# PaddlePaddle/PaddleScience

Hardware: NVIDIA H100
Metric: collocation-points/sec PDE residual loss+grad (LDC N-S) (higher is better)
Workload: dtype f32

## Files before the change

### paddlescience_b200/csrc/kernels_wgmma.cuh

```cuda
#pragma once

#include "kernels_thin.cuh"

#ifndef PPSCI_EMUL
#include <stdint.h>

namespace ppsci {
namespace wg {

constexpr int KCH = 32;
constexpr int THREADS = 256;
constexpr int TM = 64;
constexpr int A_TILE_BYTES = TM * KCH * 4;
__host__ __device__ inline int tile_points(int C) { return TM / C; }

__host__ __device__ inline int stage_bytes(int N) { return 2 * A_TILE_BYTES + 2 * N * KCH * 4; }
__host__ __device__ inline int fwd_smem_bytes(int N) { return 2 * stage_bytes(N) + 1024 + 64; }
constexpr int PREFETCH_MAX_CS = 8;

__host__ __device__ __forceinline__ uint32_t sw128(int row, int kk) {
  return (uint32_t)(row * 128 + ((((kk >> 2) ^ row) & 7) << 4) + ((kk & 3) << 2));
}
__device__ __forceinline__ uint32_t sw128_q(int row, int kq) { return (uint32_t)(row * 128 + (((kq ^ row) & 7) << 4)); }

__device__ __forceinline__ uint32_t smem_u32(const void* p) { return (uint32_t)__cvta_generic_to_shared(p); }

__device__ __forceinline__ float tf32_rn(float x) {
  uint32_t u;
  asm("cvt.rna.tf32.f32 %0, %1;" : "=r"(u) : "f"(x));
  return __uint_as_float(u);
}

__device__ __forceinline__ void mbar_init(uint32_t bar, uint32_t count) {
  asm volatile("mbarrier.init.shared::cta.b64 [%0], %1;" ::"r"(bar), "r"(count) : "memory");
}
__device__ __forceinline__ void mbar_expect_tx(uint32_t bar, uint32_t bytes) {
  asm volatile("mbarrier.arrive.expect_tx.shared::cta.b64 _, [%0], %1;" ::"r"(bar), "r"(bytes) : "memory");
}
__device__ __forceinline__ bool mbar_try_wait(uint32_t bar, uint32_t parity) {
  uint32_t ok;
  asm volatile(
      "{\n\t.reg .pred p;\n\t"
      "mbarrier.try_wait.parity.shared::cta.b64 p, [%1], %2;\n\t"
      "selp.u32 %0, 1, 0, p;\n\t}"
      : "=r"(ok)
      : "r"(bar), "r"(parity)
      : "memory");
  return ok != 0;
}
__device__ __forceinline__ void mbar_wait(uint32_t bar, uint32_t parity) {
  uint32_t spins = 0;
  while (!mbar_try_wait(bar, parity)) {
    if (++spins > (1u << 26)) __trap();
  }
}
__device__ __forceinline__ void bulk_g2s(uint32_t dst_smem, const void* src, uint32_t bytes, uint32_t bar) {
  asm volatile("cp.async.bulk.shared::cluster.global.mbarrier::complete_tx::bytes [%0], [%1], %2, [%3];" ::"r"(dst_smem),
               "l"(src), "r"(bytes), "r"(bar)
               : "memory");
}
__device__ __forceinline__ void fence_proxy_async() { asm volatile("fence.proxy.async.shared::cta;" ::: "memory"); }

__device__ __forceinline__ uint64_t make_desc(uint32_t saddr) {
  uint64_t d = 0;
  d |= (uint64_t)((saddr & 0x3FFFFu) >> 4);
  d |= (uint64_t)1 << 16;
  d |= (uint64_t)(1024 >> 4) << 32;
  d |= (uint64_t)1 << 62;
  return d;
}
__device__ __forceinline__ void wgmma_fence() { asm volatile("wgmma.fence.sync.aligned;" ::: "memory"); }
__device__ __forceinline__ void wgmma_commit() { asm volatile("wgmma.commit_group.sync.aligned;" ::: "memory"); }
template <int N>
__device__ __forceinline__ void wgmma_wait() {
  asm volatile("wgmma.wait_group.sync.aligned %0;" ::"n"(N) : "memory");
}
#define WG_T0 "%0, %1, %2, %3, %4, %5, %6, %7"
#define WG_T1 WG_T0 ", %8, %9, %10, %11, %12, %13, %14, %15"
#define WG_T2 WG_T1 ", %16, %17, %18, %19, %20, %21, %22, %23"
#define WG_T3 WG_T2 ", %24, %25, %26, %27, %28, %29, %30, %31"
#define WG_T4 WG_T3 ", %32, %33, %34, %35, %36, %37, %38, %39"
#define WG_T5 WG_T4 ", %40, %41, %42, %43, %44, %45, %46, %47"
#define WG_T6 WG_T5 ", %48, %49, %50, %51, %52, %53, %54, %55"
#define WG_T7 WG_T6 ", %56, %57, %58, %59, %60, %61, %62, %63"
#define WG_O8(b) "+f"(d[b]), "+f"(d[b + 1]), "+f"(d[b + 2]), "+f"(d[b + 3]), "+f"(d[b + 4]), "+f"(d[b + 5]), "+f"(d[b + 6]), "+f"(d[b + 7])
#define WG_O0 WG_O8(0)
#define WG_O1 WG_O0, WG_O8(8)
#define WG_O2 WG_O1, WG_O8(16)
#define WG_O3 WG_O2, WG_O8(24)
#define WG_O4 WG_O3, WG_O8(32)
#define WG_O5 WG_O4, WG_O8(40)
#define WG_O6 WG_O5, WG_O8(48)
#define WG_O7 WG_O6, WG_O8(56)
#define WG_MMA(M, G, IA, IB, IP)                                                                                  \
  __device__ __forceinline__ void wgmma_tf32(float (&d)[M / 2], uint64_t da, uint64_t db, uint32_t accumulate) { \
    asm volatile(                                                                                                 \
        "{\n\t.reg .pred p;\n\t"                                                                                  \
        "setp.ne.b32 p, %" #IP ", 0;\n\t"                                                                          \
        "wgmma.mma_async.sync.aligned.m64n" #M "k8.f32.tf32.tf32 {" WG_T##G "}, %" #IA ", %" #IB ", p, 1, 1;\n\t}"  \
        : WG_O##G                                                                                                 \
        : "l"(da), "l"(db), "r"(accumulate));                                                                     \
  }
WG_MMA(16, 0, 8, 9, 10)
WG_MMA(32, 1, 16, 17, 18)
WG_MMA(48, 2, 24, 25, 26)
WG_MMA(64, 3, 32, 33, 34)
WG_MMA(80, 4, 40, 41, 42)
WG_MMA(96, 5, 48, 49, 50)
WG_MMA(112, 6, 56, 57, 58)
WG_MMA(128, 7, 64, 65, 66)
#undef WG_MMA

__global__ void k_wg_prep_w(const float* __restrict__ W, float* __restrict__ img, int K, int N, int transposed) {
  const long long i = (long long)blockIdx.x * blockDim.x + threadIdx.x;
  if (i >= (long long)K * N) return;
  const int n = (int)(i / K), k = (int)(i % K);
  const float w = transposed ? W[(long long)n * K + k] : W[(long long)k * N + n];
  const float hi = tf32_rn(w);
  float* blk = img + (long long)(k / KCH) * 2 * N * KCH;
  const uint32_t off = sw128(n, k % KCH) >> 2;
  blk[off] = hi;
  blk[(long long)N * KCH + off] = w - hi;
}

struct WgArgs {
  AOperand<float> A;
  JetLayout J;
  const float* Wimg;
  int Kdim;
  int Kvalid;
  int Nout;
  const float* bias;
  float* Out;
  int ldo;
  long long oplane;
  long long Np;
  int num_tiles;
  const float* Zprev;
  int ldz;
  long long zplane;
  int act;
};

__device__ __forceinline__ unsigned char* xchg(unsigned char* base_ptr, int sbytes, int N, int r, int col) {
  return base_ptr + sbytes + 2 * A_TILE_BYTES + r * N * 4 + ((((col >> 2) ^ r) & 7) << 4) + (((col >> 2) & ~7) << 4) +
         (col & 3) * 4;
}

template <class L, int NQ, bool DX>
__global__ void __launch_bounds__(THREADS, 1) k_wg_layer(WgArgs g) {
  PPSCI_DYN_SMEM(smem_dyn);
  const uint32_t base = (smem_u32(smem_dyn) + 1023u) & ~1023u;
  unsigned char* base_ptr = smem_dyn + (base - smem_u32(smem_dyn));
  constexpr int CS = L::CS;
  constexpr int TP = TM / CS;
  constexpr int rows_used = CS * TP;
  constexpr int PPR = (THREADS / 32) * 4;
  constexpr int MAXI = (TP + PPR - 1) / PPR;
  constexpr int N = NQ * 32;
  constexpr int NH = N / 2;
  constexpr bool PREFETCH = CS <= PREFETCH_MAX_CS;
  const int sbytes = stage_bytes(N);
  const uint32_t bar0 = base + 2 * sbytes;
  const uint32_t b_bytes = (uint32_t)(2 * N * KCH * 4);
  const int tid = threadIdx.x, warp = tid >> 5, lane = tid & 31, wgi = tid >> 7;
  const int kq = lane & 7, psub = lane >> 3;
  const int nchunks = g.Kdim / KCH;
  const int act = g.A.act;

  if (tid == 0) {
    mbar_init(bar0, 1);
    mbar_init(bar0 + 8, 1);
    asm volatile("fence.mbarrier_init.release.cluster;" ::: "memory");
  }
  for (int s = 0; s < 2; ++s) {
    float4* az = reinterpret_cast<float4*>(base_ptr + s * sbytes);
    for (int i = tid; i < 2 * A_TILE_BYTES / 16; i += THREADS) az[i] = make_float4(0.f, 0.f, 0.f, 0.f);
  }
  fence_proxy_async();
  __syncthreads();

  float4 z[MAXI][CS];
  bool zok[MAXI];
  auto load_z = [&](int tile, int j) {
#pragma unroll
    for (int i = 0; i < MAXI; ++i) {
      const int pl = warp * 4 + psub + i * PPR;
      const long long p = (long long)tile * TP + pl;
      zok[i] = pl < TP && tile < g.num_tiles && p < g.Np;
      if (g.Kvalid && j * KCH + 4 * kq >= g.Kvalid) zok[i] = false;
      const float* src = g.A.Z + p * g.A.ld + j * KCH + 4 * kq;
#pragma unroll
      for (int c = 0; c < CS; ++c)
        z[i][c] = zok[i] ? __ldg(reinterpret_cast<const float4*>(src + (long long)c * g.A.plane)) : make_float4(0.f, 0.f, 0.f, 0.f);
    }
  };
  if constexpr (PREFETCH) load_z(blockIdx.x, 0);

  float ex[NH / 2], cr[NH / 2];
  const int rbase = (warp & 3) * 16 + (lane >> 2);
  const int cbase = wgi * NH + 2 * (lane & 3);
  uint32_t it = 0;
  for (int tile = blockIdx.x; tile < g.num_tiles; tile += gridDim.x) {
    const long long p0 = (long long)tile * TP;
#pragma unroll
    for (int e = 0; e < NH / 2; ++e) ex[e] = cr[e] = 0.f;
    for (int j = 0; j < nchunks; ++j, ++it) {
      const uint32_t s = it & 1u;
      wgmma_wait<1>();
      __syncthreads();
      const uint32_t st_addr = base + s * sbytes;
      unsigned char* st_ptr = base_ptr + s * sbytes;
      if (tid == 0) {
        mbar_expect_tx(bar0 + 8 * s, b_bytes);
        bulk_g2s(st_addr + 2 * A_TILE_BYTES, g.Wimg + (long long)j * 2 * N * KCH, b_bytes, bar0 + 8 * s);
      }
      if constexpr (!PREFETCH) load_z(tile, j);
#pragma unroll
      for (int i = 0; i < MAXI; ++i) {
        const int pl = warp * 4 + psub + i * PPR;
        if (pl >= TP) continue;
        const bool valid = zok[i];
        float yout[CS][4];
        if constexpr (DX) {
#pragma unroll
          for (int c = 0; c < CS; ++c) {
            yout[c][0] = z[i][c].x; yout[c][1] = z[i][c].y; yout[c][2] = z[i][c].z; yout[c][3] = z[i][c].w;
          }
        } else {
#pragma unroll
          for (int t = 0; t < 4; ++t) {
            auto comp = [&](const float4& v) { return t == 0 ? v.x : t == 1 ? v.y : t == 2 ? v.z : v.w; };
            float sc[6];
            float y0;
            act_coef<float, L::KM>(act, comp(z[i][0]), y0, sc);
            yout[0][t] = valid ? y0 : 0.f;
            jet_fwd<float, L>(g.J, sc, [&](int c) { return comp(z[i][c]); }, [&](int c, float v) { yout[c][t] = valid ? v : 0.f; });
          }
        }
#pragma unroll
        for (int c = 0; c < CS; ++c) {
          float4 h, l;
          h.x = tf32_rn(yout[c][0]); h.y = tf32_rn(yout[c][1]); h.z = tf32_rn(yout[c][2]); h.w = tf32_rn(yout[c][3]);
          l.x = yout[c][0] - h.x; l.y = yout[c][1] - h.y; l.z = yout[c][2] - h.z; l.w = yout[c][3] - h.w;
          const uint32_t off = sw128_q(c * TP + pl, kq);
          *reinterpret_cast<float4*>(st_ptr + off) = h;
          *reinterpret_cast<float4*>(st_ptr + A_TILE_BYTES + off) = l;
        }
      }
      if constexpr (PREFETCH) {
        if (j + 1 < nchunks) load_z(tile, j + 1);
        else load_z(tile + gridDim.x, 0);
      }
      fence_proxy_async();
      __syncthreads();
      mbar_wait(bar0 + 8 * s, (it >> 1) & 1u);
      const uint64_t a_hi = make_desc(st_addr), a_lo = make_desc(st_addr + A_TILE_BYTES);
      const uint64_t b_hi = make_desc(st_addr + 2 * A_TILE_BYTES + wgi * NH * 128), b_lo = b_hi + (uint64_t)(N * 128 / 16);
      wgmma_fence();
#pragma unroll
      for (int ks = 0; ks < KCH / 8; ++ks) {
        const uint64_t inc = (uint64_t)(2 * ks);
        const uint32_t first = (j == 0 && ks == 0) ? 0u : 1u;
        wgmma_tf32(ex, a_hi + inc, b_hi + inc, first);
        wgmma_tf32(cr, a_lo + inc, b_hi + inc, first);
        wgmma_tf32(cr, a_hi + inc, b_lo + inc, 1u);
      }
      wgmma_commit();
    }
    wgmma_wait<0>();
    if constexpr (!DX) {
#pragma unroll
      for (int h = 0; h < 2; ++h) {
        const int r = rbase + 8 * h;
        const int c = r / TP, pl = r - c * TP;
        const long long p = p0 + pl;
        if (r >= rows_used || p >= g.Np) continue;
        float* out_row = g.Out + (long long)c * g.oplane + p * g.ldo;
#pragma unroll
        for (int j = 0; j < NH / 8; ++j) {
          const int col = cbase + 8 * j;
          float2 v = make_float2(ex[4 * j + 2 * h] + cr[4 * j + 2 * h], ex[4 * j + 2 * h + 1] + cr[4 * j + 2 * h + 1]);
          if (c == 0 && g.bias) {
            v.x += __ldg(g.bias + col);
            v.y += __ldg(g.bias + col + 1);
          }
          *reinterpret_cast<float2*>(out_row + col) = v;
        }
      }
    } else {
      __syncthreads();
#pragma unroll
      for (int h = 0; h < 2; ++h) {
        const int r = rbase + 8 * h;
#pragma unroll
        for (int j = 0; j < NH / 8; ++j)
          *reinterpret_cast<float2*>(xchg(base_ptr, sbytes, N, r, cbase + 8 * j)) =
              make_float2(ex[4 * j + 2 * h] + cr[4 * j + 2 * h], ex[4 * j + 2 * h + 1] + cr[4 * j + 2 * h + 1]);
      }
      constexpr int N4 = N / 4;
      auto load_zc = [&](int item, float4 (&zc)[CS]) {
        const int pl = item / N4, q = item - pl * N4;
        const long long p = p0 + pl;
        if (item >= TP * N4 || p >= g.Np) return;
#pragma unroll
        for (int c = 0; c < CS; ++c)
          zc[c] = __ldg(reinterpret_cast<const float4*>(g.Zprev + (long long)c * g.zplane + p * g.ldz + 4 * q));
      };
      float4 znext[CS];
      if constexpr (PREFETCH) load_zc(tid, znext);
      __syncthreads();
      for (int item = tid; item < TP * N4; item += THREADS) {
        const int pl = item / N4, q = item - pl * N4;
        const long long p = p0 + pl;
        float4 zc[CS];
        if constexpr (PREFETCH) {
#pragma unroll
          for (int c = 0; c < CS; ++c) zc[c] = znext[c];
          load_zc(item + THREADS, znext);
        } else {
          load_zc(item, zc);
        }
        if (p >= g.Np) continue;
        float4 xc[CS];
#pragma unroll
        for (int c = 0; c < CS; ++c) xc[c] = *reinterpret_cast<const float4*>(xchg(base_ptr, sbytes, N, c * TP + pl, 4 * q));
        float ob[CS][4];
#pragma unroll
        for (int t = 0; t < 4; ++t) {
          auto comp = [&](const float4& v) { return t == 0 ? v.x : t == 1 ? v.y : t == 2 ? v.z : v.w; };
          float sc[6];
          float y0;
          act_coef<float, L::KM + 1>(g.act, comp(zc[0]), y0, sc);
          ob[0][t] = jet_adj<float, L>(g.J, sc, [&](int c) { return comp(zc[c]); }, [&](int c) { return comp(xc[c]); },
                                       [&](int c, float v) { ob[c][t] = v; });
        }
        float* out = g.Out + p * g.ldo + 4 * q;
#pragma unroll
        for (int c = 0; c < CS; ++c)
          *reinterpret_cast<float4*>(out + (long long)c * g.oplane) = make_float4(ob[c][0], ob[c][1], ob[c][2], ob[c][3]);
      }
      fence_proxy_async();
      __syncthreads();
    }
  }
}

__host__ __device__ constexpr int dw_pch(int C) { return C >= 8 ? 4 : C >= 3 ? 8 : 32 / C; }
__host__ __device__ constexpr int dw_groups(int C) { return dw_pch(C) / 4 * C; }
__host__ __device__ constexpr int dw_ksteps(int C) { return (dw_groups(C) + 1) / 2; }
__host__ __device__ constexpr int dw_atoms(int C) { return (dw_ksteps(C) + 3) / 4; }
__host__ __device__ constexpr int dw_maxq(int C) { return C <= 5 ? 4 : C <= 8 ? 2 : 1; }
__host__ __device__ constexpr int dw_smem_bytes(int C, int bnq) {
  return 2 * 2 * dw_atoms(C) * bnq * 32 * 128 + bnq * 32 * 4 + dw_pch(C) / 4 * 2 * C * 256 * 4 + bnq * 32 * 2 * 256 + 1024;
}
constexpr int DW_TK = 128;
constexpr int DW_FLUSH_ROWS = 512;
__host__ __device__ constexpr int dw_flush(int C) {
  return DW_FLUSH_ROWS / (dw_pch(C) * C) > 1 ? DW_FLUSH_ROWS / (dw_pch(C) * C) : 1;
}

struct WgDwArgs {
  AOperand<float> A;
  JetLayout J;
  const float* Zbar;
  int ldzb;
  long long zbplane;
  int Kdim;
  int Nout;
  int col_blocks;
  float* dW;
  float* db;
  long long Np;
  int chunks_per_split;
};

__device__ __forceinline__ void wgmma_tf32_rA_m64n64(float (&d)[32], const uint32_t (&a)[4], uint64_t db) {
  asm volatile(
      "{\n\t.reg .pred p;\n\t"
      "setp.ne.b32 p, %37, 0;\n\t"
      "wgmma.mma_async.sync.aligned.m64n64k8.f32.tf32.tf32 "
      "{%0, %1, %2, %3, %4, %5, %6, %7, %8, %9, %10, %11, %12, %13, %14, %15, "
      "%16, %17, %18, %19, %20, %21, %22, %23, %24, %25, %26, %27, %28, %29, %30, %31}, "
      "{%32, %33, %34, %35}, %36, p, 1, 1;\n\t}"
      : "+f"(d[0]), "+f"(d[1]), "+f"(d[2]), "+f"(d[3]), "+f"(d[4]), "+f"(d[5]), "+f"(d[6]), "+f"(d[7]), "+f"(d[8]),
        "+f"(d[9]), "+f"(d[10]), "+f"(d[11]), "+f"(d[12]), "+f"(d[13]), "+f"(d[14]), "+f"(d[15]), "+f"(d[16]),
        "+f"(d[17]), "+f"(d[18]), "+f"(d[19]), "+f"(d[20]), "+f"(d[21]), "+f"(d[22]), "+f"(d[23]), "+f"(d[24]),
        "+f"(d[25]), "+f"(d[26]), "+f"(d[27]), "+f"(d[28]), "+f"(d[29]), "+f"(d[30]), "+f"(d[31])
      : "r"(a[0]), "r"(a[1]), "r"(a[2]), "r"(a[3]), "l"(db), "r"(1u));
}
__device__ __forceinline__ void wgmma_tf32_rA_m64n32(float (&d)[16], const uint32_t (&a)[4], uint64_t db) {
  asm volatile(
      "{\n\t.reg .pred p;\n\t"
      "setp.ne.b32 p, %21, 0;\n\t"
      "wgmma.mma_async.sync.aligned.m64n32k8.f32.tf32.tf32 "
      "{%0, %1, %2, %3, %4, %5, %6, %7, %8, %9, %10, %11, %12, %13, %14, %15}, "
      "{%16, %17, %18, %19}, %20, p, 1, 1;\n\t}"
      : "+f"(d[0]), "+f"(d[1]), "+f"(d[2]), "+f"(d[3]), "+f"(d[4]), "+f"(d[5]), "+f"(d[6]), "+f"(d[7]), "+f"(d[8]),
        "+f"(d[9]), "+f"(d[10]), "+f"(d[11]), "+f"(d[12]), "+f"(d[13]), "+f"(d[14]), "+f"(d[15])
      : "r"(a[0]), "r"(a[1]), "r"(a[2]), "r"(a[3]), "l"(db), "r"(1u));
}

template <class L, int BNQ>
__global__ void __launch_bounds__(THREADS, 1) k_wg_dw(WgDwArgs g) {
  PPSCI_DYN_SMEM(smem_dyn);
  const uint32_t base = (smem_u32(smem_dyn) + 1023u) & ~1023u;
  unsigned char* base_ptr = smem_dyn + (base - smem_u32(smem_dyn));
  constexpr int CS = L::CS, PCH = dw_pch(CS), QPC = PCH / 4, G = dw_groups(CS), KS = dw_ksteps(CS), NA = dw_atoms(CS);
  constexpr int BN = BNQ * 32, NB = BNQ / 2, TAIL = BNQ & 1;
  constexpr int ATOM = BN * 128;
  constexpr int STAGE = 2 * NA * ATOM;
  constexpr int BI = (G * BN + THREADS - 1) / THREADS;
  const int tid = threadIdx.x, warp = tid >> 5, lane = tid & 31, wgi = tid >> 7, t = lane & 3;
  const int kb = blockIdx.x / g.col_blocks, n0 = (blockIdx.x - kb * g.col_blocks) * BN;
  const int Np = (int)g.Np;
  const int total_chunks = (Np + PCH - 1) / PCH;
  const int ch_begin = blockIdx.y * g.chunks_per_split;
  const int ch_end = ch_begin + g.chunks_per_split < total_chunks ? ch_begin + g.chunks_per_split : total_chunks;
  if (ch_begin >= ch_end) return;
  const int act = g.A.act;
  const int krow = kb * DW_TK + wgi * 64 + (warp & 3) * 16 + (lane >> 2);

  float* bsum = reinterpret_cast<float*>(base_ptr + 2 * STAGE);
  for (int i = tid; i < (2 * STAGE + BN * 4) / 16; i += THREADS)
    reinterpret_cast<float4*>(base_ptr)[i] = make_float4(0.f, 0.f, 0.f, 0.f);
  __syncthreads();

  float ex[NB > 0 ? NB : 1][32], ext[TAIL ? 16 : 1], cr[NB > 0 ? NB : 1][32], crt[TAIL ? 16 : 1];
#pragma unroll
  for (int nb = 0; nb < NB; ++nb)
#pragma unroll
    for (int i = 0; i < 32; ++i) ex[nb][i] = cr[nb][i] = 0.f;
#pragma unroll
  for (int i = 0; i < (TAIL ? 16 : 1); ++i) ext[i] = crt[i] = 0.f;

  auto acc_at = [&](int e) -> float {
    return e < 32 * NB ? ex[e >> 5][e & 31] + cr[e >> 5][e & 31] : ext[e - 32 * NB] + crt[e - 32 * NB];
  };
  float4* part = reinterpret_cast<float4*>(base_ptr + 2 * STAGE + BN * 4 + QPC * 2 * CS * THREADS * 4);
#pragma unroll
  for (int q = 0; q < BN / 8; ++q) part[q * THREADS + tid] = make_float4(0.f, 0.f, 0.f, 0.f);
  auto flush = [&]() {
#pragma unroll
    for (int q = 0; q < BN / 8; ++q) {
      float4 p = part[q * THREADS + tid];
      p.x += acc_at(4 * q); p.y += acc_at(4 * q + 1); p.z += acc_at(4 * q + 2); p.w += acc_at(4 * q + 3);
      part[q * THREADS + tid] = p;
    }
#pragma unroll
    for (int nb = 0; nb < NB; ++nb)
#pragma unroll
      for (int i = 0; i < 32; ++i) ex[nb][i] = cr[nb][i] = 0.f;
#pragma unroll
    for (int i = 0; i < (TAIL ? 16 : 1); ++i) ext[i] = crt[i] = 0.f;
  };

  float* za = reinterpret_cast<float*>(base_ptr + 2 * STAGE + BN * 4);
  auto za_at = [&](int qq, int h, int c) -> float* { return za + ((qq * 2 + h) * CS + c) * THREADS + tid; };
  float4 zb[BI];
  auto load_a = [&](int ch) {
    const int p0 = ch * PCH;
#pragma unroll
    for (int qq = 0; qq < QPC; ++qq)
#pragma unroll
      for (int h = 0; h < 2; ++h) {
        const int p = p0 + 4 * qq + t;
        const int k = krow + 8 * h;
        const bool ok = p < Np && k < g.Kdim;
        const float* src = g.A.Z + (ok ? (long long)p * g.A.ld + k : 0);
#pragma unroll
        for (int c = 0; c < CS; ++c)
          asm volatile("cp.async.ca.shared.global [%0], [%1], 4, %2;" ::"r"(smem_u32(za_at(qq, h, c))),
                       "l"(src + (ok ? (long long)c * g.A.plane : 0)), "r"(ok ? 4 : 0)
                       : "memory");
      }
    asm volatile("cp.async.commit_group;" ::: "memory");
  };
  auto load_b = [&](int ch) {
    const int p0 = ch * PCH;
#pragma unroll
    for (int i = 0; i < BI; ++i) {
      const int item = tid + THREADS * i;
      const int gi = item / BN, n = item - gi * BN;
      const int qq = gi / CS, c = gi - qq * CS;
      const int p = p0 + 4 * qq;
      const bool ok = item < G * BN && n0 + n < g.Nout;
      const float* src = g.Zbar + (long long)c * g.zbplane + (long long)p * g.ldzb + n0 + n;
      zb[i].x = ok && p < Np ? __ldg(src) : 0.f;
      zb[i].y = ok && p + 1 < Np ? __ldg(src + g.ldzb) : 0.f;
      zb[i].z = ok && p + 2 < Np ? __ldg(src + 2 * g.ldzb) : 0.f;
      zb[i].w = ok && p + 3 < Np ? __ldg(src + 3 * g.ldzb) : 0.f;
    }
  };

  load_a(ch_begin);
  load_b(ch_begin);
  uint32_t ahi[KS][4], alo[KS][4];
  for (int ch = ch_begin; ch < ch_end; ++ch) {
    const int sidx = (ch - ch_begin) & 1;
    const uint32_t st_addr = base + sidx * STAGE;
    unsigned char* st = base_ptr + sidx * STAGE;
#pragma unroll
    for (int i = 0; i < BI; ++i) {
      const int item = tid + THREADS * i;
      if (item >= G * BN) continue;
      const int gi = item / BN, n = item - gi * BN;
      const float4 v = zb[i];
      float4 hi, lo;
      hi.x = tf32_rn(v.x); hi.y = tf32_rn(v.y); hi.z = tf32_rn(v.z); hi.w = tf32_rn(v.w);
      lo.x = v.x - hi.x; lo.y = v.y - hi.y; lo.z = v.z - hi.z; lo.w = v.w - hi.w;
      const uint32_t off = (gi >> 3) * ATOM + sw128_q(n, gi & 7);
      *reinterpret_cast<float4*>(st + off) = hi;
      *reinterpret_cast<float4*>(st + NA * ATOM + off) = lo;
      if (kb == 0 && gi % CS == 0) atomicAdd(bsum + n, (v.x + v.y) + (v.z + v.w));
    }
    wgmma_wait<0>();
    if (ch > ch_begin && (ch - ch_begin) % dw_flush(CS) == 0) flush();
    asm volatile("cp.async.wait_group 0;" ::: "memory");
    float av[QPC][2][CS];
#pragma unroll
    for (int qq = 0; qq < QPC; ++qq)
#pragma unroll
      for (int h = 0; h < 2; ++h) {
        float z[CS], sc[6];
#pragma unroll
        for (int c = 0; c < CS; ++c) z[c] = *za_at(qq, h, c);
        act_coef<float, L::KM>(act, z[0], av[qq][h][0], sc);
        jet_fwd<float, L>(g.J, sc, [&](int c) { return z[c]; }, [&](int c, float v) { av[qq][h][c] = v; });
      }
    if (ch + 1 < ch_end) load_a(ch + 1);
    fence_proxy_async();
    __syncthreads();
#pragma unroll
    for (int s = 0; s < KS; ++s)
#pragma unroll
      for (int e = 0; e < 2; ++e)
#pragma unroll
        for (int h = 0; h < 2; ++h) {
          const int gi = 2 * s + e;
          const float v = gi < G ? av[gi / CS][h][gi % CS] : 0.f;
          const float vh = tf32_rn(v);
          ahi[s][2 * e + h] = __float_as_uint(vh);
          alo[s][2 * e + h] = __float_as_uint(v - vh);
        }
    wgmma_fence();
#pragma unroll
    for (int s = 0; s < KS; ++s) {
      const uint64_t b_hi = make_desc(st_addr + (s >> 2) * ATOM + (s & 3) * 32);
      const uint64_t b_lo = b_hi + (uint64_t)(NA * ATOM / 16);
#pragma unroll
      for (int nb = 0; nb < NB; ++nb) {
        const uint64_t bo = (uint64_t)(nb * 64 * 128 / 16);
        wgmma_tf32_rA_m64n64(ex[nb], ahi[s], b_hi + bo);
        wgmma_tf32_rA_m64n64(cr[nb], alo[s], b_hi + bo);
        wgmma_tf32_rA_m64n64(cr[nb], ahi[s], b_lo + bo);
      }
      if constexpr (TAIL) {
        const uint64_t bo = (uint64_t)(NB * 64 * 128 / 16);
        wgmma_tf32_rA_m64n32(ext, ahi[s], b_hi + bo);
        wgmma_tf32_rA_m64n32(crt, alo[s], b_hi + bo);
        wgmma_tf32_rA_m64n32(crt, ahi[s], b_lo + bo);
      }
    }
    wgmma_commit();
    if (ch + 1 < ch_end) load_b(ch + 1);
  }
  wgmma_wait<0>();
#pragma unroll
  for (int h = 0; h < 2; ++h) {
    const int k = krow + 8 * h;
    if (k >= g.Kdim) continue;
    float* row = g.dW + (long long)k * g.Nout + n0;
#pragma unroll
    for (int j = 0; j < BN / 8; ++j) {
      if (n0 + 8 * j >= g.Nout) break;
      const int col = 8 * j + 2 * t;
      const float4 p = part[j * THREADS + tid];
      atomicAdd(row + col, (h ? p.z : p.x) + acc_at(4 * j + 2 * h));
      atomicAdd(row + col + 1, (h ? p.w : p.y) + acc_at(4 * j + 2 * h + 1));
    }
  }
  if (kb == 0) {
    __syncthreads();
    if (tid < BN && n0 + tid < g.Nout) atomicAdd(g.db + n0 + tid, bsum[tid]);
  }
}

}

inline int wg_kpad(int K) { return (K + wg::KCH - 1) / wg::KCH * wg::KCH; }
inline bool wg_shape_ok(int K, int N) { return K % wg::KCH == 0 && K >= 32 && K <= 1024 && N % 32 == 0 && N >= 32 && N <= 256; }
inline bool wg_plan_ok(const ppsci_plan_spec& s, const JetLayout& J) {
  return s.dtype == PPSCI_F32 && !s.gated && !act_has_param(s.act) && with_lay(WgLays{}, J, [](auto) {});
}
inline bool wg_fwd_ok(const ppsci_plan_spec& s, int l) {
  if (l == 1) return s.dense_in && s.n_layers >= 2 && s.widths[0] % 4 == 0 && wg_shape_ok(wg_kpad(s.widths[0]), s.widths[1]);
  if (l < 2 || l > s.n_layers) return false;
  return wg_shape_ok(s.widths[l - 1], s.widths[l]);
}
inline bool wg_dx_ok(const ppsci_plan_spec& s, int l) {
  if (l < 2 || l > s.n_layers) return false;
  return wg_shape_ok(s.widths[l], s.widths[l - 1]);
}

inline bool wg_dw_ok(const ppsci_plan_spec& s, int l) {
  if (l < 1 || (l == 1 && !s.dense_in) || l > s.n_layers) return false;
  const int K = s.widths[l - 1], N = s.widths[l];
  return K % 4 == 0 && N % 32 == 0 && N >= 32 && N <= 256;
}

}
#endif
```

Baseline: 5.808 million.

## Stage dW A-operand in swizzled smem and overlap wgmma with next-chunk loads

Reworks the weight-gradient wgmma kernel so the activation-jet A operand is computed from register-prefetched loads and written to shared memory in a 32-byte swizzled layout. Both A and B are now read by wgmma through smem descriptors instead of the A operand coming from registers via cp.async scalar copies. The main loop double-buffers stages and waits with wait_group<1>, so the next chunk's global loads and transforms can overlap the in-flight MMAs. The cost is more shared-memory traffic and staging, and a different accumulator layout using one full-width N tile.

New measurement: 5.977 million, median of 6. +2.9%, better.

```diff
diff --git a/paddlescience_b200/csrc/kernels_wgmma.cuh b/paddlescience_b200/csrc/kernels_wgmma.cuh
--- a/paddlescience_b200/csrc/kernels_wgmma.cuh
+++ b/paddlescience_b200/csrc/kernels_wgmma.cuh
@@ -69,6 +69,15 @@
   d |= (uint64_t)1 << 62;
   return d;
 }
+__device__ __forceinline__ uint64_t make_desc_sw32(uint32_t saddr) {
+  uint64_t d = 0;
+  d |= (uint64_t)((saddr & 0x3FFFFu) >> 4);
+  d |= (uint64_t)1 << 16;
+  d |= (uint64_t)(256 >> 4) << 32;
+  d |= (uint64_t)3 << 62;
+  return d;
+}
+__device__ __forceinline__ uint32_t sw32_q(int row, int h) { return (uint32_t)(row * 32 + (((h ^ (row >> 2)) & 1) << 4)); }
 __device__ __forceinline__ void wgmma_fence() { asm volatile("wgmma.fence.sync.aligned;" ::: "memory"); }
 __device__ __forceinline__ void wgmma_commit() { asm volatile("wgmma.commit_group.sync.aligned;" ::: "memory"); }
 template <int N>
@@ -349,12 +358,12 @@
 __host__ __device__ constexpr int dw_pch(int C) { return C >= 8 ? 4 : C >= 3 ? 8 : 32 / C; }
 __host__ __device__ constexpr int dw_groups(int C) { return dw_pch(C) / 4 * C; }
 __host__ __device__ constexpr int dw_ksteps(int C) { return (dw_groups(C) + 1) / 2; }
-__host__ __device__ constexpr int dw_atoms(int C) { return (dw_ksteps(C) + 3) / 4; }
 __host__ __device__ constexpr int dw_maxq(int C) { return C <= 5 ? 4 : C <= 8 ? 2 : 1; }
+constexpr int DW_TK = 128;
+__host__ __device__ constexpr int dw_stage_bytes(int C, int bnq) { return 2 * dw_ksteps(C) * (DW_TK + bnq * 32) * 32; }
 __host__ __device__ constexpr int dw_smem_bytes(int C, int bnq) {
-  return 2 * 2 * dw_atoms(C) * bnq * 32 * 128 + bnq * 32 * 4 + dw_pch(C) / 4 * 2 * C * 256 * 4 + bnq * 32 * 2 * 256 + 1024;
-}
-constexpr int DW_TK = 128;
+  return 2 * dw_stage_bytes(C, bnq) + bnq * 32 * 4 + bnq * 32 * 2 * 256 + 1024;
+}
 constexpr int DW_FLUSH_ROWS = 512;
 __host__ __device__ constexpr int dw_flush(int C) {
   return DW_FLUSH_ROWS / (dw_pch(C) * C) > 1 ? DW_FLUSH_ROWS / (dw_pch(C) * C) : 1;
@@ -375,41 +384,17 @@
   int chunks_per_split;
 };
 
-__device__ __forceinline__ void wgmma_tf32_rA_m64n64(float (&d)[32], const uint32_t (&a)[4], uint64_t db) {
-  asm volatile(
-      "{\n\t.reg .pred p;\n\t"
-      "setp.ne.b32 p, %37, 0;\n\t"
-      "wgmma.mma_async.sync.aligned.m64n64k8.f32.tf32.tf32 "
-      "{%0, %1, %2, %3, %4, %5, %6, %7, %8, %9, %10, %11, %12, %13, %14, %15, "
-      "%16, %17, %18, %19, %20, %21, %22, %23, %24, %25, %26, %27, %28, %29, %30, %31}, "
-      "{%32, %33, %34, %35}, %36, p, 1, 1;\n\t}"
-      : "+f"(d[0]), "+f"(d[1]), "+f"(d[2]), "+f"(d[3]), "+f"(d[4]), "+f"(d[5]), "+f"(d[6]), "+f"(d[7]), "+f"(d[8]),
-        "+f"(d[9]), "+f"(d[10]), "+f"(d[11]), "+f"(d[12]), "+f"(d[13]), "+f"(d[14]), "+f"(d[15]), "+f"(d[16]),
-        "+f"(d[17]), "+f"(d[18]), "+f"(d[19]), "+f"(d[20]), "+f"(d[21]), "+f"(d[22]), "+f"(d[23]), "+f"(d[24]),
-        "+f"(d[25]), "+f"(d[26]), "+f"(d[27]), "+f"(d[28]), "+f"(d[29]), "+f"(d[30]), "+f"(d[31])
-      : "r"(a[0]), "r"(a[1]), "r"(a[2]), "r"(a[3]), "l"(db), "r"(1u));
-}
-__device__ __forceinline__ void wgmma_tf32_rA_m64n32(float (&d)[16], const uint32_t (&a)[4], uint64_t db) {
-  asm volatile(
-      "{\n\t.reg .pred p;\n\t"
-      "setp.ne.b32 p, %21, 0;\n\t"
-      "wgmma.mma_async.sync.aligned.m64n32k8.f32.tf32.tf32 "
-      "{%0, %1, %2, %3, %4, %5, %6, %7, %8, %9, %10, %11, %12, %13, %14, %15}, "
-      "{%16, %17, %18, %19}, %20, p, 1, 1;\n\t}"
-      : "+f"(d[0]), "+f"(d[1]), "+f"(d[2]), "+f"(d[3]), "+f"(d[4]), "+f"(d[5]), "+f"(d[6]), "+f"(d[7]), "+f"(d[8]),
-        "+f"(d[9]), "+f"(d[10]), "+f"(d[11]), "+f"(d[12]), "+f"(d[13]), "+f"(d[14]), "+f"(d[15])
-      : "r"(a[0]), "r"(a[1]), "r"(a[2]), "r"(a[3]), "l"(db), "r"(1u));
-}
-
 template <class L, int BNQ>
 __global__ void __launch_bounds__(THREADS, 1) k_wg_dw(WgDwArgs g) {
   PPSCI_DYN_SMEM(smem_dyn);
   const uint32_t base = (smem_u32(smem_dyn) + 1023u) & ~1023u;
   unsigned char* base_ptr = smem_dyn + (base - smem_u32(smem_dyn));
-  constexpr int CS = L::CS, PCH = dw_pch(CS), QPC = PCH / 4, G = dw_groups(CS), KS = dw_ksteps(CS), NA = dw_atoms(CS);
-  constexpr int BN = BNQ * 32, NB = BNQ / 2, TAIL = BNQ & 1;
-  constexpr int ATOM = BN * 128;
-  constexpr int STAGE = 2 * NA * ATOM;
+  constexpr int CS = L::CS, PCH = dw_pch(CS), QPC = PCH / 4, G = dw_groups(CS), KS = dw_ksteps(CS);
+  constexpr int BN = BNQ * 32;
+  constexpr int AK = DW_TK * 32, BK = BN * 32;
+  constexpr int B_OFF = 2 * KS * AK;
+  constexpr int STAGE = dw_stage_bytes(CS, BNQ);
+  constexpr int AI = (DW_TK * QPC + THREADS - 1) / THREADS;
   constexpr int BI = (G * BN + THREADS - 1) / THREADS;
   const int tid = threadIdx.x, warp = tid >> 5, lane = tid & 31, wgi = tid >> 7, t = lane & 3;
   const int kb = blockIdx.x / g.col_blocks, n0 = (blockIdx.x - kb * g.col_blocks) * BN;
@@ -424,60 +409,44 @@
   float* bsum = reinterpret_cast<float*>(base_ptr + 2 * STAGE);
   for (int i = tid; i < (2 * STAGE + BN * 4) / 16; i += THREADS)
     reinterpret_cast<float4*>(base_ptr)[i] = make_float4(0.f, 0.f, 0.f, 0.f);
-  __syncthreads();
-
-  float ex[NB > 0 ? NB : 1][32], ext[TAIL ? 16 : 1], cr[NB > 0 ? NB : 1][32], crt[TAIL ? 16 : 1];
-#pragma unroll
-  for (int nb = 0; nb < NB; ++nb)
-#pragma unroll
-    for (int i = 0; i < 32; ++i) ex[nb][i] = cr[nb][i] = 0.f;
-#pragma unroll
-  for (int i = 0; i < (TAIL ? 16 : 1); ++i) ext[i] = crt[i] = 0.f;
-
-  auto acc_at = [&](int e) -> float {
-    return e < 32 * NB ? ex[e >> 5][e & 31] + cr[e >> 5][e & 31] : ext[e - 32 * NB] + crt[e - 32 * NB];
-  };
-  float4* part = reinterpret_cast<float4*>(base_ptr + 2 * STAGE + BN * 4 + QPC * 2 * CS * THREADS * 4);
+
+  float ex[BN / 2], cr[BN / 2];
+#pragma unroll
+  for (int i = 0; i < BN / 2; ++i) ex[i] = cr[i] = 0.f;
+  float4* part = reinterpret_cast<float4*>(base_ptr + 2 * STAGE + BN * 4);
 #pragma unroll
   for (int q = 0; q < BN / 8; ++q) part[q * THREADS + tid] = make_float4(0.f, 0.f, 0.f, 0.f);
   auto flush = [&]() {
 #pragma unroll
     for (int q = 0; q < BN / 8; ++q) {
       float4 p = part[q * THREADS + tid];
-      p.x += acc_at(4 * q); p.y += acc_at(4 * q + 1); p.z += acc_at(4 * q + 2); p.w += acc_at(4 * q + 3);
+      p.x += ex[4 * q] + cr[4 * q]; p.y += ex[4 * q + 1] + cr[4 * q + 1];
+      p.z += ex[4 * q + 2] + cr[4 * q + 2]; p.w += ex[4 * q + 3] + cr[4 * q + 3];
       part[q * THREADS + tid] = p;
     }
 #pragma unroll
-    for (int nb = 0; nb < NB; ++nb)
-#pragma unroll
-      for (int i = 0; i < 32; ++i) ex[nb][i] = cr[nb][i] = 0.f;
-#pragma unroll
-    for (int i = 0; i < (TAIL ? 16 : 1); ++i) ext[i] = crt[i] = 0.f;
+    for (int i = 0; i < BN / 2; ++i) ex[i] = cr[i] = 0.f;
   };
 
-  float* za = reinterpret_cast<float*>(base_ptr + 2 * STAGE + BN * 4);
-  auto za_at = [&](int qq, int h, int c) -> float* { return za + ((qq * 2 + h) * CS + c) * THREADS + tid; };
-  float4 zb[BI];
-  auto load_a = [&](int ch) {
+  float4 za[AI][CS], zb[BI];
+  auto load = [&](int ch) {
     const int p0 = ch * PCH;
 #pragma unroll
-    for (int qq = 0; qq < QPC; ++qq)
-#pragma unroll
-      for (int h = 0; h < 2; ++h) {
-        const int p = p0 + 4 * qq + t;
-        const int k = krow + 8 * h;
-        const bool ok = p < Np && k < g.Kdim;
-        const float* src = g.A.Z + (ok ? (long long)p * g.A.ld + k : 0);
-#pragma unroll
-        for (int c = 0; c < CS; ++c)
-          asm volatile("cp.async.ca.shared.global [%0], [%1], 4, %2;" ::"r"(smem_u32(za_at(qq, h, c))),
-                       "l"(src + (ok ? (long long)c * g.A.plane : 0)), "r"(ok ? 4 : 0)
-                       : "memory");
-      }
-    asm volatile("cp.async.commit_group;" ::: "memory");
-  };
-  auto load_b = [&](int ch) {
-    const int p0 = ch * PCH;
+    for (int i = 0; i < AI; ++i) {
+      const int item = tid + THREADS * i;
+      const int qq = item / DW_TK, k = kb * DW_TK + item - qq * DW_TK;
+      const int p = p0 + 4 * qq;
+      const bool ok = item < DW_TK * QPC && k < g.Kdim;
+      const float* src = g.A.Z + (long long)p * g.A.ld + k;
+#pragma unroll
+      for (int c = 0; c < CS; ++c) {
+        const float* s = src + (long long)c * g.A.plane;
+        za[i][c].x = ok && p < Np ? __ldg(s) : 0.f;
+        za[i][c].y = ok && p + 1 < Np ? __ldg(s + g.A.ld) : 0.f;
+        za[i][c].z = ok && p + 2 < Np ? __ldg(s + 2 * g.A.ld) : 0.f;
+        za[i][c].w = ok && p + 3 < Np ? __ldg(s + 3 * g.A.ld) : 0.f;
+      }
+    }
 #pragma unroll
     for (int i = 0; i < BI; ++i) {
       const int item = tid + THREADS * i;
@@ -492,14 +461,31 @@
       zb[i].w = ok && p + 3 < Np ? __ldg(src + 3 * g.ldzb) : 0.f;
     }
   };
-
-  load_a(ch_begin);
-  load_b(ch_begin);
-  uint32_t ahi[KS][4], alo[KS][4];
-  for (int ch = ch_begin; ch < ch_end; ++ch) {
-    const int sidx = (ch - ch_begin) & 1;
-    const uint32_t st_addr = base + sidx * STAGE;
-    unsigned char* st = base_ptr + sidx * STAGE;
+  auto store = [&](unsigned char* st) {
+#pragma unroll
+    for (int i = 0; i < AI; ++i) {
+      const int item = tid + THREADS * i;
+      if (item >= DW_TK * QPC) continue;
+      const int qq = item / DW_TK, r = item - qq * DW_TK;
+      float av[CS][4];
+#pragma unroll
+      for (int u = 0; u < 4; ++u) {
+        auto comp = [&](const float4& v) { return u == 0 ? v.x : u == 1 ? v.y : u == 2 ? v.z : v.w; };
+        float sc[6];
+        act_coef<float, L::KM>(act, comp(za[i][0]), av[0][u], sc);
+        jet_fwd<float, L>(g.J, sc, [&](int c) { return comp(za[i][c]); }, [&](int c, float v) { av[c][u] = v; });
+      }
+#pragma unroll
+      for (int c = 0; c < CS; ++c) {
+        const int gi = c + CS * qq;
+        float4 hi, lo;
+        hi.x = tf32_rn(av[c][0]); hi.y = tf32_rn(av[c][1]); hi.z = tf32_rn(av[c][2]); hi.w = tf32_rn(av[c][3]);
+        lo.x = av[c][0] - hi.x; lo.y = av[c][1] - hi.y; lo.z = av[c][2] - hi.z; lo.w = av[c][3] - hi.w;
+        const uint32_t off = (gi >> 1) * AK + sw32_q(r, gi & 1);
+        *reinterpret_cast<float4*>(st + off) = hi;
+        *reinterpret_cast<float4*>(st + KS * AK + off) = lo;
+      }
+    }
 #pragma unroll
     for (int i = 0; i < BI; ++i) {
       const int item = tid + THREADS * i;
@@ -509,61 +495,37 @@
       float4 hi, lo;
       hi.x = tf32_rn(v.x); hi.y = tf32_rn(v.y); hi.z = tf32_rn(v.z); hi.w = tf32_rn(v.w);
       lo.x = v.x - hi.x; lo.y = v.y - hi.y; lo.z = v.z - hi.z; lo.w = v.w - hi.w;
-      const uint32_t off = (gi >> 3) * ATOM + sw128_q(n, gi & 7);
+      const uint32_t off = B_OFF + (gi >> 1) * BK + sw32_q(n, gi & 1);
       *reinterpret_cast<float4*>(st + off) = hi;
-      *reinterpret_cast<float4*>(st + NA * ATOM + off) = lo;
+      *reinterpret_cast<float4*>(st + KS * BK + off) = lo;
       if (kb == 0 && gi % CS == 0) atomicAdd(bsum + n, (v.x + v.y) + (v.z + v.w));
     }
-    wgmma_wait<0>();
-    if (ch > ch_begin && (ch - ch_begin) % dw_flush(CS) == 0) flush();
-    asm volatile("cp.async.wait_group 0;" ::: "memory");
-    float av[QPC][2][CS];
-#pragma unroll
-    for (int qq = 0; qq < QPC; ++qq)
-#pragma unroll
-      for (int h = 0; h < 2; ++h) {
-        float z[CS], sc[6];
-#pragma unroll
-        for (int c = 0; c < CS; ++c) z[c] = *za_at(qq, h, c);
-        act_coef<float, L::KM>(act, z[0], av[qq][h][0], sc);
-        jet_fwd<float, L>(g.J, sc, [&](int c) { return z[c]; }, [&](int c, float v) { av[qq][h][c] = v; });
-      }
-    if (ch + 1 < ch_end) load_a(ch + 1);
+  };
+
+  load(ch_begin);
+  for (int ch = ch_begin; ch < ch_end; ++ch) {
+    const int sidx = (ch - ch_begin) & 1;
+    const uint32_t st_addr = base + sidx * STAGE;
+    wgmma_wait<1>();
+    __syncthreads();
+    store(base_ptr + sidx * STAGE);
+    if (ch + 1 < ch_end) load(ch + 1);
     fence_proxy_async();
     __syncthreads();
-#pragma unroll
-    for (int s = 0; s < KS; ++s)
-#pragma unroll
-      for (int e = 0; e < 2; ++e)
-#pragma unroll
-        for (int h = 0; h < 2; ++h) {
-          const int gi = 2 * s + e;
-          const float v = gi < G ? av[gi / CS][h][gi % CS] : 0.f;
-          const float vh = tf32_rn(v);
-          ahi[s][2 * e + h] = __float_as_uint(vh);
-          alo[s][2 * e + h] = __float_as_uint(v - vh);
-        }
+    if (ch > ch_begin && (ch - ch_begin) % dw_flush(CS) == 0) {
+      wgmma_wait<0>();
+      flush();
+    }
     wgmma_fence();
 #pragma unroll
     for (int s = 0; s < KS; ++s) {
-      const uint64_t b_hi = make_desc(st_addr + (s >> 2) * ATOM + (s & 3) * 32);
-      const uint64_t b_lo = b_hi + (uint64_t)(NA * ATOM / 16);
-#pragma unroll
-      for (int nb = 0; nb < NB; ++nb) {
-        const uint64_t bo = (uint64_t)(nb * 64 * 128 / 16);
-        wgmma_tf32_rA_m64n64(ex[nb], ahi[s], b_hi + bo);
-        wgmma_tf32_rA_m64n64(cr[nb], alo[s], b_hi + bo);
-        wgmma_tf32_rA_m64n64(cr[nb], ahi[s], b_lo + bo);
-      }
-      if constexpr (TAIL) {
-        const uint64_t bo = (uint64_t)(NB * 64 * 128 / 16);
-        wgmma_tf32_rA_m64n32(ext, ahi[s], b_hi + bo);
-        wgmma_tf32_rA_m64n32(crt, alo[s], b_hi + bo);
-        wgmma_tf32_rA_m64n32(crt, ahi[s], b_lo + bo);
-      }
+      const uint64_t a_hi = make_desc_sw32(st_addr + s * AK + wgi * 64 * 32), a_lo = a_hi + (uint64_t)(KS * AK / 16);
+      const uint64_t b_hi = make_desc_sw32(st_addr + B_OFF + s * BK), b_lo = b_hi + (uint64_t)(KS * BK / 16);
+      wgmma_tf32(ex, a_hi, b_hi, 1u);
+      wgmma_tf32(cr, a_lo, b_hi, 1u);
+      wgmma_tf32(cr, a_hi, b_lo, 1u);
     }
     wgmma_commit();
-    if (ch + 1 < ch_end) load_b(ch + 1);
   }
   wgmma_wait<0>();
 #pragma unroll
@@ -575,9 +537,10 @@
     for (int j = 0; j < BN / 8; ++j) {
       if (n0 + 8 * j >= g.Nout) break;
       const int col = 8 * j + 2 * t;
+      const int e = 4 * j + 2 * h;
       const float4 p = part[j * THREADS + tid];
-      atomicAdd(row + col, (h ? p.z : p.x) + acc_at(4 * j + 2 * h));
-      atomicAdd(row + col + 1, (h ? p.w : p.y) + acc_at(4 * j + 2 * h + 1));
+      atomicAdd(row + col, (h ? p.z : p.x) + (ex[e] + cr[e]));
+      atomicAdd(row + col + 1, (h ? p.w : p.y) + (ex[e + 1] + cr[e + 1]));
     }
   }
   if (kb == 0) {
```
